# AppleHolic/pytorch_sound

Measured on AMD Instinct MI355X. Metric: audio-sec/s STFT+mel+fwd/bwd, higher is better.
Workload: dtype bf16; 1 GPU; configs[1]: Conv1d separator (4 x ResBlock1, C=256, on 513-bin magnitude), 22.05 kHz, STFT 1024/256, 80 mel, batch 32 x 2 s per GPU, Adam, bf16 autocast; global_batch=32, parallelism=dp1, model_params=5520386

## Files before the change

### include/psnd.h

```cpp
#ifndef PSND_H
#define PSND_H

#include <stdint.h>
#include <stddef.h>

#ifdef __cplusplus
extern "C" {
#endif

#define PSND_OK 0
#define PSND_E_ARG (-1)
#define PSND_E_SHAPE (-2)
#define PSND_E_HIP (-3)
#define PSND_E_UNSUPPORTED (-4)

#define PSND_FRAMING_CENTER 0
#define PSND_FRAMING_HIFIGAN 1
#define PSND_FRAMING_NONE 2

int psnd_version(void);
const char *psnd_last_error(void);
#ifdef PSND_LAB
void psnd_env_refresh(void);
#endif
// ... 65 lines not shown
typedef struct psnd_chain_pair {
    const void *W1;
    const float *bias1;
    float act1_slope;
    void *mid_out;
    const void *W2;
    const float *bias2;
    int off1, dstep1, off2, dstep2;
    float act2_slope;
    void *out_raw, *out_act;
    const void *M1, *M2;
    float m1_slope, m2_slope;
} psnd_chain_pair;
int psnd_conv1d_cl_chain_rows(int C, int k, int n_pairs, const int *taps);
int psnd_conv1d_cl_chain_plan(int C, int k, int n_pairs, const int *taps, int64_t R, int *mr_out);
int psnd_conv1d_cl_chain(const void *A, const void *res, const psnd_chain_pair *pairs, int n_pairs, int64_t N, int Lp, int L, int HP,
                         int C, int k, void *stream);
void psnd_conv_chain_stats(long long *out2);
int psnd_to_cl_nfk(const float *x_nfk, int64_t N, int K, int64_t F, int Lp, int HP, int Cp, int preop, void *out, void *stream);
int64_t psnd_mask_head_l1_blocks_nfk(int64_t N, int64_t F, int K);
int psnd_mask_head_l1_fwd_nfk(const void *y, const float *mag_nfk, const float *ref_nfk, int64_t N, int K, int64_t F, int Lp, int HP, int Cp,
                              float *est_nfk, double *part, void *stream);
int psnd_mask_head_l1_bwd_nfk(const float *gest_nfk, const float *mag_nfk, const void *y, const float *est_nfk, const float *ref_nfk,
                              const float *g, float coef, int64_t N, int K, int64_t F, int Lp, int HP, int Cp, void *gy, void *stream);
int psnd_mel_fwd_nfk(const float *mag_nfk, int64_t N, int64_t F, int M, int K, const void *mel_plan, int log_kind, float log_offset,
                     float pre_clamp_min, float clamp_lo, float clamp_hi, float *out, float *mel_lin, void *stream);
int psnd_mel_bwd_nfk(const float *gout, const float *mel_lin, int64_t N, int64_t F, int M, int K, const void *mel_plan, int log_kind,
                     float log_offset, float pre_clamp_min, float clamp_lo, float clamp_hi, float *gmag_nfk, void *stream);
int psnd_mel_l1_fwd_nfk(const float *mag_nfk, int64_t N, int64_t F, int M, int K, const void *mel_plan, int log_kind, float log_offset,
                        float pre_clamp_min, float clamp_lo, float clamp_hi, const float *ref, float *mel_lin, double *part, void *stream);
int psnd_mel_l1_bwd_nfk(const float *ref, const float *mel_lin, const float *g, float coef, int64_t N, int64_t F, int M, int K,
                        const void *mel_plan, int log_kind, float log_offset, float pre_clamp_min, float clamp_lo, float clamp_hi,
                        float *gmag_nfk, void *stream);
int64_t psnd_mask_head_l1_blocks(int64_t N, int64_t T, int Cp);
int psnd_mask_head_l1_fwd(const void *y, const float *mag, const float *ref, int64_t N, int C, int64_t T, int Lp, int HP, int Cp,
                          float *est, double *part, void *stream);
int psnd_mask_head_l1_bwd(const float *gest, const float *mag, const void *y, const float *est, const float *ref, const float *g,
                          float coef, int64_t N, int C, int64_t T, int Lp, int HP, int Cp, void *gy, void *stream);
int64_t psnd_mel_l1_blocks(int64_t N, int64_t F, int M);
int psnd_mel_l1_fwd(const float *mag, int64_t N, int64_t F, int M, int K, const void *mel_plan, int log_kind, float log_offset,
                    float pre_clamp_min, float clamp_lo, float clamp_hi, const float *ref, float *mel_lin, double *part, void *stream);
int psnd_mel_l1_bwd(const float *ref, const float *mel_lin, const float *g, float coef, int64_t N, int64_t F, int M, int K,
                    const void *mel_plan, int log_kind, float log_offset, float pre_clamp_min, float clamp_lo, float clamp_hi,
                    float *gmag, void *stream);
int psnd_nan_flag(const float *x, int64_t n, float *flag, void *stream);
int psnd_l1_loss_combine(const double *const *parts, const int64_t *nb, const double *scale, int terms, float *out, float *nan_flag, void *stream);
int psnd_conv_stats(int64_t *out4, int reset);
int psnd_conv_pair_stats(int64_t *out4, int reset);
int psnd_conv1d_cl_wgrad(const void *G1, const void *G2, const void *GM, float g2_slope, const void *xa, int64_t N,
                         int Lp, int Ca, int Cb, int k, int off0, int dstep, float *gw_part, float *gbias_part,
                         void *g_out, void *stream);
int psnd_conv1d_prep(const float *v, const float *g, const float *bias, int Cout, int Cin, int k, int Cb, int Ca,
                     void *wf, void *wb, float *bias_padded, void *stream);
int psnd_convtr1d_prep(const float *v, const float *g, const float *bias, int Cin, int Cout, int K, int stride, int Cr, int Cip,
                       void *wf, void *wb, float *bias_rep, void *stream);
int psnd_convtr1d_prep_multi(const void *descs_dev, int n, int total_blocks, void *stream);
int psnd_convtr1d_cl_fwd(const void *xa, const void *wf, const float *bias_rep, int64_t N, int Lp, int L, int HP, int Cip, int Cr,
                         int stride, int padding, int LpO, int HPO, float act_slope, void *out_raw, void *out_act, void *stream);
int psnd_convtr1d_cl_wgrad_splits(int64_t N, int Lp, int Cip, int Cr, int stride);
int psnd_convtr1d_cl_bwd(const void *g_raw, const void *g_act, const void *act, float act_slope, const void *wb, const void *xa,
                         int64_t N, int Lp, int L, int HP, int Cip, int Cr, int stride, int padding, int LpO, int HPO, void *gx,
                         void *g_eff, float *gw_part, void *stream);
int psnd_convtr1d_wnorm_bwd(const float *gw_part, int splits, const float *v, const float *g, int Cin, int Cout, int K, int stride,
                            int Cr, int Cip, float *gv, float *gg, void *stream);
int psnd_cl_mean_act_fwd(const void *a, const void *b, const void *c, const void *d, int count, float slope, void *out, int64_t n,
                         void *stream);
// ... 162 lines not shown
```

### pytorch_sound_amd/_lib.py

```python
import ctypes
import os
import numpy as np

_HERE = os.path.dirname(os.path.abspath(__file__))
LIB_PATH = os.environ.get('PSND_LIB', os.path.join(_HERE, 'libpsnd_hip.so'))

PSND_OK = 0
FRAMING_CENTER = 0
FRAMING_HIFIGAN = 1
FRAMING_NONE = 2
LOG_NONE, LOG_E, LOG_10 = 0, 1, 2

_c = ctypes
_P = _c.c_void_p
_I64 = _c.c_int64
_INT = _c.c_int
_F = _c.c_float
_D = _c.c_double
_U32 = _c.c_uint32
_U64 = _c.c_uint64

SIGNATURES = {
    'psnd_version': (_INT, []),
    'psnd_last_error': (_c.c_char_p, []),
# ... 18 lines not shown
    'psnd_conv1d_cl': (_INT, [_P, _P, _P, _F, _P, _P, _P, _P, _I64, _INT, _INT, _INT, _INT, _INT, _INT, _INT, _INT, _F, _F, _P, _P, _P, _P]),
    'psnd_conv1d_cl_pair_supported': (_INT, [_INT, _INT, _INT, _INT, _INT, _INT]),
    'psnd_conv1d_cl_pair': (_INT, [_P, _P, _P, _P, _F, _F, _P, _P, _P, _P, _F, _P, _I64, _INT, _INT, _INT, _INT, _INT, _INT, _INT, _INT, _INT, _F, _P, _P, _P]),
    'psnd_conv1d_cl_wgrad': (_INT, [_P, _P, _P, _F, _P, _I64, _INT, _INT, _INT, _INT, _INT, _INT, _P, _P, _P, _P]),
    'psnd_conv1d_prep': (_INT, [_P, _P, _P, _INT, _INT, _INT, _INT, _INT, _P, _P, _P, _P]),
    'psnd_conv1d_wnorm_bwd': (_INT, [_P, _P, _INT, _P, _P, _INT, _INT, _INT, _INT, _INT, _P, _P, _P, _P]),
    'psnd_conv1d_cl_bwd': (_INT, [_P, _P, _P, _F, _P, _P, _I64, _INT, _INT, _INT, _INT, _INT, _INT, _INT, _INT, _P, _P, _P, _F, _P, _P, _P, _P]),
    'psnd_conv1d_cl_wgrad_multi_splits': (_INT, [_I64, _INT, _INT, _INT, _INT, _INT]),
    'psnd_conv1d_cl_wgrad_multi': (_INT, [_P, _INT, _I64, _INT, _P]),
    'psnd_nan_flag': (_INT, [_P, _I64, _P, _P]),
    'psnd_conv1d_cl_chain_rows': (_INT, [_INT, _INT, _INT, _P]),
    'psnd_conv1d_cl_chain_plan': (_INT, [_INT, _INT, _INT, _P, _I64, _P]),
    'psnd_conv1d_cl_chain': (_INT, [_P, _P, _P, _INT, _I64, _INT, _INT, _INT, _INT, _INT, _P]),
    'psnd_conv_chain_stats': (None, [_P]),
    'psnd_conv1d_cl_pair_bwd_supported': (_INT, [_INT, _INT, _INT, _INT, _INT, _INT]),
    'psnd_conv1d_cl_pair_bwd_splits': (_INT, [_I64, _INT, _INT, _INT]),
    'psnd_conv1d_cl_pair_bwd': (_INT, [_P, _P, _P, _F, _P, _P, _P, _F, _P, _I64, _INT, _INT, _INT, _INT, _INT, _INT, _INT, _INT, _INT, _P, _P, _P, _P,
                                       _P, _P, _INT, _INT, _P, _P, _P]),
    'psnd_conv1d_wnorm_bwd_multi': (_INT, [_P, _INT, _P]),
    'psnd_conv1d_prep_multi': (_INT, [_P, _INT, _INT, _INT, _INT, _P]),
    'psnd_conv1d_cl_wgrad_splits': (_INT, [_I64, _INT, _INT, _INT, _INT]),
    'psnd_mask_head_l1_blocks': (_I64, [_I64, _I64, _INT]),
    'psnd_masked_l1_blocks': (_I64, [_I64]),
    'psnd_masked_l1_fwd': (_INT, [_P, _P, _P, _I64, _INT, _I64, _P, _P, _P, _P]),
    'psnd_masked_l1_bwd': (_INT, [_P, _P, _P, _I64, _INT, _I64, _P, _P, _P, _P, _P]),
    'psnd_to_cl_nfk': (_INT, [_P, _I64, _INT, _I64, _INT, _INT, _INT, _INT, _P, _P]),
    'psnd_mask_head_l1_blocks_nfk': (_I64, [_I64, _I64, _INT]),
    'psnd_mask_head_l1_fwd_nfk': (_INT, [_P, _P, _P, _I64, _INT, _I64, _INT, _INT, _INT, _P, _P, _P]),
    'psnd_mask_head_l1_bwd_nfk': (_INT, [_P, _P, _P, _P, _P, _P, _F, _I64, _INT, _I64, _INT, _INT, _INT, _P, _P]),
    'psnd_mel_fwd_nfk': (_INT, [_P, _I64, _I64, _INT, _INT, _P, _INT, _F, _F, _F, _F, _P, _P, _P]),
    'psnd_mel_bwd_nfk': (_INT, [_P, _P, _I64, _I64, _INT, _INT, _P, _INT, _F, _F, _F, _F, _P, _P]),
    'psnd_mel_l1_fwd_nfk': (_INT, [_P, _I64, _I64, _INT, _INT, _P, _INT, _F, _F, _F, _F, _P, _P, _P, _P]),
    'psnd_mel_l1_bwd_nfk': (_INT, [_P, _P, _P, _F, _I64, _I64, _INT, _INT, _P, _INT, _F, _F, _F, _F, _P, _P]),
    'psnd_mask_head_l1_fwd': (_INT, [_P, _P, _P, _I64, _INT, _I64, _INT, _INT, _INT, _P, _P, _P]),
    'psnd_mask_head_l1_bwd': (_INT, [_P, _P, _P, _P, _P, _P, _F, _I64, _INT, _I64, _INT, _INT, _INT, _P, _P]),
    'psnd_mel_l1_blocks': (_I64, [_I64, _I64, _INT]),
    'psnd_mel_l1_fwd': (_INT, [_P, _I64, _I64, _INT, _INT, _P, _INT, _F, _F, _F, _F, _P, _P, _P, _P]),
    'psnd_mel_l1_bwd': (_INT, [_P, _P, _P, _F, _I64, _I64, _INT, _INT, _P, _INT, _F, _F, _F, _F, _P, _P]),
    'psnd_l1_loss_combine': (_INT, [_P, _P, _P, _INT, _P, _P, _P]),
    'psnd_conv_stats': (_INT, [_P, _INT]),
    'psnd_conv_pair_stats': (_INT, [_P, _INT]),
    'psnd_convtr1d_prep_multi': (_INT, [_P, _INT, _INT, _P]),
    'psnd_convtr1d_prep': (_INT, [_P, _P, _P, _INT, _INT, _INT, _INT, _INT, _INT, _P, _P, _P, _P]),
    'psnd_convtr1d_cl_fwd': (_INT, [_P, _P, _P, _I64, _INT, _INT, _INT, _INT, _INT, _INT, _INT, _INT, _INT, _F, _P, _P, _P]),
    'psnd_convtr1d_cl_wgrad_splits': (_INT, [_I64, _INT, _INT, _INT, _INT]),
    'psnd_convtr1d_cl_bwd': (_INT, [_P, _P, _P, _F, _P, _P, _I64, _INT, _INT, _INT, _INT, _INT, _INT, _INT, _INT, _INT, _P, _P, _P, _P]),
    'psnd_convtr1d_wnorm_bwd': (_INT, [_P, _INT, _P, _P, _INT, _INT, _INT, _INT, _INT, _INT, _P, _P, _P]),
    'psnd_cl_mean_act_fwd': (_INT, [_P, _P, _P, _P, _INT, _F, _P, _I64, _P]),
    'psnd_cl_mean_act_bwd': (_INT, [_P, _P, _INT, _F, _P, _I64, _P]),
    'psnd_cl_sum2': (_INT, [_P, _INT, _P, _P, _INT, _P, _I64, _P]),
    'psnd_grad_pack_bf16': (_INT, [_P, _P, _I64, _F, _P]),
    'psnd_grad_unpack_bf16': (_INT, [_P, _P, _I64, _F, _P]),
    'psnd_cl_colsum_splits': (_INT, [_I64, _INT]),
    'psnd_cl_colsum': (_INT, [_P, _I64, _INT, _INT, _INT, _INT, _P, _P, _P]),
    'psnd_posenc': (_INT, [_P, _P, _F, _I64, _INT, _I64, _I64, _P, _P]),
    'psnd_groupnorm1_fwd': (_INT, [_P, _P, _P, _P, _I64, _INT, _I64, _F, _INT, _P, _P, _P, _P]),
    'psnd_groupnorm1_bwd': (_INT, [_P, _P, _P, _P, _P, _P, _I64, _INT, _I64, _INT, _P, _P, _P, _P, _P]),
    'psnd_groupnorm1_drop_fwd': (_INT, [_P, _P, _P, _P, _I64, _INT, _I64, _F, _INT, _P, _P, _P, _P, _U32, _F, _P]),
    'psnd_groupnorm1_drop_bwd': (_INT, [_P, _P, _P, _P, _P, _P, _I64, _INT, _I64, _INT, _P, _P, _P, _P, _P, _P, _U32, _F, _P]),
    'psnd_rng_seed': (_INT, [_P, _U64, _U64, _P]),
    'psnd_rng_next': (_INT, [_P, _P, _P]),
    'psnd_linear1x1_fwd': (_INT, [_P, _P, _P, _I64, _INT, _INT, _I64, _INT, _INT, _P, _P]),
    'psnd_linear1x1_wgrad_slabs': (_I64, [_I64, _INT, _INT, _I64]),
    'psnd_linear1x1_bwd': (_INT, [_P, _P, _P, _P, _I64, _INT, _INT, _I64, _INT, _P, _P, _P, _P, _P]),
    'psnd_linear1x1_bwd_acc': (_INT, [_P, _P, _P, _P, _I64, _INT, _INT, _I64, _INT, _P, _P, _P, _P, _P, _P]),
    'psnd_linear1x1_bwd_ex': (_INT, [_P, _P, _P, _P, _I64, _INT, _INT, _I64, _INT, _INT, _I64, _P, _P, _P, _P, _P, _P, _P]),
# ... 172 lines not shown
```

### pytorch_sound_amd/cl.py

```python
import ctypes
import os
from pytorch_sound_amd import _switches as _sw
import weakref

import torch

from . import _lib
from ._lib import lib, check, ptr, stream_ptr

ALIGN_C = 32


def round_up(x, m):
    return (x + m - 1) // m * m


class CLShape:

    def __init__(self, N, L, HP):
        self.N, self.L, self.HP = int(N), int(L), int(HP)
        self.Lp = round_up(self.L + 2 * self.HP, 8)

    @property
    def R(self):
# ... 168 lines not shown
    def backward(ctx, g, _gest):
        y, mag, mag_ref, mel_ref, mel_plan, est, lin = ctx.saved_tensors
        shape, M, log_kind, log_offset, pre, lo, hi, c1, c2 = ctx.cfg
        N, C, T = mag.shape
        if g is None:
            return (None,) * 14
        g = g.contiguous().float()
        gest = torch.empty_like(mag)
        gy = torch.empty_like(y)
        st = stream_ptr(y.device)
        with torch.cuda.device(y.device):
            check(lib().psnd_mel_l1_bwd(ptr(mel_ref), ptr(lin), ptr(g), c2, N, T, M, C, ptr(mel_plan), log_kind, log_offset, pre, lo, hi,
                                        ptr(gest), st), 'psnd_mel_l1_bwd')
            check(lib().psnd_mask_head_l1_bwd(ptr(gest), ptr(mag), ptr(y), ptr(est), ptr(mag_ref), ptr(g), c1, N, C, T, shape.Lp, shape.HP,
                                              y.shape[2], ptr(gy), st), 'psnd_mask_head_l1_bwd')
        return (gy,) + (None,) * 13


def to_cl_nfk(x_nfk, shape, preop=0):
    _need(x_nfk, torch.float32)
    if x_nfk.requires_grad and torch.is_grad_enabled():
        raise _lib.PsndError('to_cl_nfk carries no gradient (feature tensors are inputs); use ToCL on an (N, K, F) tensor')
    N, F, K = x_nfk.shape
    if F != shape.L or N != shape.N:
        raise _lib.PsndError('to_cl_nfk: tensor %s does not match the CL geometry (N=%d, L=%d)' % (tuple(x_nfk.shape), shape.N, shape.L))
    Cp = round_up(K, ALIGN_C)
    out = torch.empty((N, shape.Lp, Cp), dtype=torch.bfloat16, device=x_nfk.device)
    with torch.cuda.device(x_nfk.device):
        check(lib().psnd_to_cl_nfk(ptr(x_nfk), N, K, F, shape.Lp, shape.HP, Cp, int(preop), ptr(out), stream_ptr(x_nfk.device)),
              'psnd_to_cl_nfk')
    return out


class MaskHeadSpectralL1NFK(torch.autograd.Function):

    @staticmethod
    def forward(ctx, y, mag, mag_ref, mel_ref, mel_plan, shape, M, log_kind, log_offset, pre_clamp_min, clamp_lo, clamp_hi, w1, w2):
        from .kernels import _clamp_args
        ctx.set_materialize_grads(False)
        _need(y, torch.bfloat16)
        for t in (mag, mag_ref, mel_ref):
            _need(t, torch.float32)
        N, F, K = mag.shape
        if mag_ref.shape != mag.shape or tuple(mel_ref.shape) != (N, M, F):
            raise _lib.PsndError('mask_head_spectral_l1 (nfk): mag_ref %s / mel_ref %s do not match mag %s and %d mel bands'
                                 % (tuple(mag_ref.shape), tuple(mel_ref.shape), tuple(mag.shape), M))
        dev = y.device
        lo, hi, pre = _clamp_args(clamp_lo, clamp_hi, pre_clamp_min)
        est = torch.empty_like(mag)
        lin = torch.empty((N, M, F), dtype=torch.float32, device=dev)
        nb1 = int(lib().psnd_mask_head_l1_blocks_nfk(N, F, K))
        nb2 = int(lib().psnd_mel_l1_blocks(N, F, M))
        part = torch.empty(nb1 + nb2, dtype=torch.float64, device=dev)
        out = torch.empty((), dtype=torch.float32, device=dev)
        st = stream_ptr(dev)
        with torch.cuda.device(dev):
            check(lib().psnd_mask_head_l1_fwd_nfk(ptr(y), ptr(mag), ptr(mag_ref), N, K, F, shape.Lp, shape.HP, y.shape[2], ptr(est),
                                                  ptr(part), st), 'psnd_mask_head_l1_fwd_nfk')
            p2 = ctypes.c_void_p(part.data_ptr() + 8 * nb1)
            check(lib().psnd_mel_l1_fwd_nfk(ptr(est), N, F, M, K, ptr(mel_plan), log_kind, float(log_offset), pre, lo, hi, ptr(mel_ref),
                                            ptr(lin), p2, st), 'psnd_mel_l1_fwd_nfk')
            parts = (ctypes.c_void_p * 2)(part.data_ptr(), part.data_ptr() + 8 * nb1)
            nbs = (ctypes.c_int64 * 2)(nb1, nb2)
            sc = (ctypes.c_double * 2)(float(w1) / mag.numel(), float(w2) / mel_ref.numel())
            nan_flag = _nan_flag_tensor(dev)
            check(lib().psnd_l1_loss_combine(parts, nbs, sc, 2, ptr(out), ptr(nan_flag), st), 'psnd_l1_loss_combine')
        LAST_LOSS_NAN_FLAG[0] = nan_flag
        ctx.cfg = (shape, M, log_kind, float(log_offset), pre, lo, hi, float(w1) / mag.numel(), float(w2) / mel_ref.numel())
        ctx.save_for_backward(y, mag, mag_ref, mel_ref, mel_plan, est, lin)
        ctx.mark_non_differentiable(est)
        return out, est

    @staticmethod
    def backward(ctx, g, _gest):
        y, mag, mag_ref, mel_ref, mel_plan, est, lin = ctx.saved_tensors
        shape, M, log_kind, log_offset, pre, lo, hi, c1, c2 = ctx.cfg
        N, F, K = mag.shape
        if g is None:
            return (None,) * 14
        g = g.contiguous().float()
        gest = torch.empty_like(mag)
        gy = torch.empty_like(y)
        st = stream_ptr(y.device)
        with torch.cuda.device(y.device):
            check(lib().psnd_mel_l1_bwd_nfk(ptr(mel_ref), ptr(lin), ptr(g), c2, N, F, M, K, ptr(mel_plan), log_kind, log_offset, pre, lo, hi,
                                            ptr(gest), st), 'psnd_mel_l1_bwd_nfk')
            check(lib().psnd_mask_head_l1_bwd_nfk(ptr(gest), ptr(mag), ptr(y), ptr(est), ptr(mag_ref), ptr(g), c1, N, K, F, shape.Lp,
                                                  shape.HP, y.shape[2], ptr(gy), st), 'psnd_mask_head_l1_bwd_nfk')
        return (gy,) + (None,) * 13


def _launch_conv(A, A2, AM, a2_slope, W, bias, res, mask_src, shape, Ca, Cb, k, off0, dstep, act_slope, mask_slope,
                 want_raw, want_act, a_eff_out=None):
    dev = W.device
    raw = torch.empty((shape.N, shape.Lp, Cb), dtype=torch.bfloat16, device=dev) if want_raw else None
    act = torch.empty((shape.N, shape.Lp, Cb), dtype=torch.bfloat16, device=dev) if want_act else None
    with torch.cuda.device(dev):
        check(lib().psnd_conv1d_cl(ptr(A), ptr(A2), ptr(AM), float(a2_slope), ptr(W), ptr(bias), ptr(res), ptr(mask_src),
                                   shape.N, shape.Lp, shape.L, shape.HP, Ca, Cb, k, off0, dstep, float(act_slope),
                                   float(mask_slope), ptr(raw), ptr(act), ptr(a_eff_out), stream_ptr(dev)), 'psnd_conv1d_cl')
    return raw, act


_JOIN_PENDING = {}


def _join_side_at_end_of_backward(dev, side):
    target = torch.cuda.current_stream(dev)
    pending = _JOIN_PENDING.setdefault(dev.index, [])
    if not any(t == target and sd == side for t, sd in pending):
        pending.append((target, side))

    def join():
        for t, sd in _JOIN_PENDING.pop(dev.index, []):
            t.wait_stream(sd)

# ... 1019 lines not shown
```

### pytorch_sound_amd/csrc/psnd_core.hip

```cpp
#include "psnd_common.h"

static thread_local char g_err[512] = "";

void psnd_set_error(const char *fmt, ...) {
    va_list ap;
    va_start(ap, fmt);
    vsnprintf(g_err, sizeof(g_err), fmt, ap);
    va_end(ap);
}

extern "C" int psnd_version(void) { return 140; }

extern "C" const char *psnd_last_error(void) { return g_err; }

#ifdef PSND_LAB
std::atomic<int> g_psnd_env_gen{0};
extern "C" void psnd_env_refresh(void) { g_psnd_env_gen.fetch_add(1, std::memory_order_acq_rel); }
#endif

static inline int64_t pad_of(int n_fft, int hop, int framing) {
    if (framing == PSND_FRAMING_NONE) return 0;
    return framing == PSND_FRAMING_CENTER ? n_fft / 2 : (n_fft - hop) / 2;
}

extern "C" int64_t psnd_frame_count(int64_t T, int n_fft, int hop, int framing) {
    if (T <= 0 || n_fft <= 0 || hop <= 0) return 0;
    const int64_t L = T + 2 * pad_of(n_fft, hop, framing);
    if (L < n_fft) return 0;
    return (L - n_fft) / hop + 1;
}

extern "C" int64_t psnd_frame_sample_index(int64_t f, int m, int64_t T, int n_fft, int hop, int framing) {
    int64_t i = f * hop - pad_of(n_fft, hop, framing) + m;
    if (i < 0) i = -i;
    if (i >= T) i = 2 * (T - 1) - i;
    return i;
}

extern "C" void *psnd_event_create(void) {
    hipEvent_t ev = nullptr;
    if (hipEventCreateWithFlags(&ev, hipEventDisableTiming) != hipSuccess) {
        psnd_set_error("event_create: %s", hipGetErrorString(hipGetLastError()));
        return nullptr;
    }
// ... 96 lines not shown
```

### pytorch_sound_amd/csrc/psnd_mel.hip

```cpp
#include "psnd_common.h"
#include <math.h>
#include <string.h>
#include <vector>

namespace {

inline int hdr_ints(int MT, int KT) { return (8 + 2 * MT + 2 * KT + 63) & ~63; }

struct MelParams {
    const float *in0;
    const float *in1;
    const int *plan;
    float *out;
    float *lin;
    long long F;
    int N, R, Cc;
    int RT, CS;
    int band_off;
    int w_off;
    int nft;
    int log_kind;
    float log_offset, pre_clamp_min, clamp_lo, clamp_hi;
    const float *l1_ref;
    double *l1_part;
// ... 292 lines not shown
                        const f32x4 rf = *reinterpret_cast<const f32x4_u *>(p.l1_ref + o);
                        l1acc += fabsf(y.x - rf.x) + fabsf(y.y - rf.y) + fabsf(y.z - rf.z) + fabsf(y.w - rf.w);
                        *reinterpret_cast<f32x4_u *>(p.lin + o) = v;
                    } else {
                        for (int j = 0; j < 4; ++j)
                            if (f + j < F) {
                                l1acc += fabsf(y[j] - p.l1_ref[o + j]);
                                p.lin[o + j] = v[j];
                            }
                    }
                    continue;
                }
                if (f + 3 < F) {
                    *reinterpret_cast<f32x4_u *>(p.out + o) = y;
                    if (p.lin) *reinterpret_cast<f32x4_u *>(p.lin + o) = v;
                } else {
                    for (int j = 0; j < 4; ++j)
                        if (f + j < F) {
                            p.out[o + j] = y[j];
                            if (p.lin) p.lin[o + j] = v[j];
                        }
                }
            }
            if (p.l1_part) {
                double d = (double)l1acc;
#pragma unroll
                for (int m = 32; m >= 1; m >>= 1) d += __shfl_xor(d, m, 64);
                if (lane == 0) p.l1_part[wid * p.RT + T] = d;
            }
        }
    });
}

struct MelHostPlan {
    int M, K, MT, KS, KT, MS, hdr, fw_off, bw_off, wn_off, KS16, seg_off;
    size_t total_bytes;
};
MelHostPlan mel_layout(int M, int K) {
    MelHostPlan h;
    h.M = M, h.K = K;
    h.MT = (M + 15) / 16, h.KS = (K + 3) / 4;
    h.KT = (K + 15) / 16, h.MS = (M + 3) / 4;
    h.hdr = hdr_ints(h.MT, h.KT);
    h.fw_off = h.hdr;
    h.bw_off = h.fw_off + h.MT * h.KS * 64;
    h.KS16 = (K + 15) / 16;
    h.wn_off = h.bw_off + h.KT * h.MS * 64;
    h.seg_off = h.wn_off + h.MT * h.KS16 * 256;
    h.total_bytes = sizeof(float) * ((size_t)h.seg_off + 4 * h.MT + 4);
    return h;
}

}

extern "C" size_t psnd_mel_plan_bytes(int M, int K) {
    if (M <= 0 || K <= 0) return 0;
    return mel_layout(M, K).total_bytes;
}

extern "C" int psnd_mel_plan_build(int M, int K, const float *W, void *plan_host) {
    if (!W || !plan_host || M <= 0 || K <= 0) PSND_FAIL(PSND_E_ARG, "mel_plan_build: bad arguments");
    const MelHostPlan h = mel_layout(M, K);
    memset(plan_host, 0, h.total_bytes);
    int *hdr = static_cast<int *>(plan_host);
    float *fl = static_cast<float *>(plan_host);
    hdr[0] = M, hdr[1] = K, hdr[2] = h.MT, hdr[3] = h.KS, hdr[4] = h.KT, hdr[5] = h.MS;
// ... 126 lines not shown
}
extern "C" int psnd_mel_l1_bwd(const float *ref, const float *mel_lin, const float *g, float coef, int64_t N, int64_t F, int M, int K,
                               const void *mel_plan, int log_kind, float log_offset, float pre_clamp_min, float clamp_lo, float clamp_hi,
                               float *gmag, void *stream) {
    if (!g) PSND_FAIL(PSND_E_ARG, "mel_l1_bwd: null g");
    return mel_launch(true, ref, mel_lin, N, F, M, K, mel_plan, log_kind, log_offset, pre_clamp_min, clamp_lo, clamp_hi, gmag, nullptr,
                      stream, nullptr, nullptr, g, coef);
}

extern "C" int psnd_mel_fwd_nfk(const float *mag_nfk, int64_t N, int64_t F, int M, int K, const void *mel_plan, int log_kind, float log_offset,
                                float pre_clamp_min, float clamp_lo, float clamp_hi, float *out, float *mel_lin, void *stream) {
    return mel_launch(false, mag_nfk, nullptr, N, F, M, K, mel_plan, log_kind, log_offset, pre_clamp_min, clamp_lo, clamp_hi, out, mel_lin, stream,
                      nullptr, nullptr, nullptr, 0.f, true);
}
extern "C" int psnd_mel_bwd_nfk(const float *gout, const float *mel_lin, int64_t N, int64_t F, int M, int K, const void *mel_plan, int log_kind,
                                float log_offset, float pre_clamp_min, float clamp_lo, float clamp_hi, float *gmag_nfk, void *stream) {
    return mel_launch(true, gout, mel_lin, N, F, M, K, mel_plan, log_kind, log_offset, pre_clamp_min, clamp_lo, clamp_hi, gmag_nfk, nullptr, stream,
                      nullptr, nullptr, nullptr, 0.f, true);
}
extern "C" int psnd_mel_l1_fwd_nfk(const float *mag_nfk, int64_t N, int64_t F, int M, int K, const void *mel_plan, int log_kind, float log_offset,
                                   float pre_clamp_min, float clamp_lo, float clamp_hi, const float *ref, float *mel_lin, double *part,
                                   void *stream) {
    if (!ref || !mel_lin || !part) PSND_FAIL(PSND_E_ARG, "mel_l1_fwd_nfk: null ref / mel_lin / part");
    return mel_launch(false, mag_nfk, nullptr, N, F, M, K, mel_plan, log_kind, log_offset, pre_clamp_min, clamp_lo, clamp_hi, nullptr, mel_lin,
                      stream, ref, part, nullptr, 0.f, true);
}
extern "C" int psnd_mel_l1_bwd_nfk(const float *ref, const float *mel_lin, const float *g, float coef, int64_t N, int64_t F, int M, int K,
                                   const void *mel_plan, int log_kind, float log_offset, float pre_clamp_min, float clamp_lo, float clamp_hi,
                                   float *gmag_nfk, void *stream) {
    if (!g) PSND_FAIL(PSND_E_ARG, "mel_l1_bwd_nfk: null g");
    return mel_launch(true, ref, mel_lin, N, F, M, K, mel_plan, log_kind, log_offset, pre_clamp_min, clamp_lo, clamp_hi, gmag_nfk, nullptr,
                      stream, nullptr, nullptr, g, coef, true);
}
```

Before: 96750 audio-s/s.

## Fuse mask head, spectral L1, mel projection and mel L1 into single fwd/bwd kernels

Adds fused forward and backward kernels covering the mask-head sigmoid, the spectral L1 loss, the mel MFMA projection with log/clamp and the mel L1 loss. The forward kernel also does the final loss reduction and combine through a last-block ticket counter. This replaces several separate launches and the intermediate est/gest round-trips through memory with one launch per direction. The cost is more complex kernels with redundant overlapping loads, per-stream ticket state that must stay correct across calls, and a per-wave double reduction.

```diff
diff --git a/include/psnd.h b/include/psnd.h
--- a/include/psnd.h
+++ b/include/psnd.h
@@ -121,6 +121,15 @@
 int psnd_mel_l1_bwd_nfk(const float *ref, const float *mel_lin, const float *g, float coef, int64_t N, int64_t F, int M, int K,
                         const void *mel_plan, int log_kind, float log_offset, float pre_clamp_min, float clamp_lo, float clamp_hi,
                         float *gmag_nfk, void *stream);
+int64_t psnd_mask_mel_l1_parts(int64_t N, int64_t F, int M);
+int psnd_mask_mel_l1_fwd_nfk(const void *y, const float *mag_nfk, const float *ref_nfk, const float *mel_ref, int64_t N, int K, int64_t F, int M,
+                             int Lp, int HP, int Cp, const void *mel_plan, int log_kind, float log_offset, float pre_clamp_min, float clamp_lo,
+                             float clamp_hi, double scale1, double scale2, float *est_nfk, float *mel_lin, double *part, unsigned *ticket,
+                             float *out, float *nan_flag, void *stream);
+int psnd_mask_mel_l1_bwd_nfk(const float *mag_nfk, const void *y, const float *est_nfk, const float *ref_nfk, const float *mel_ref,
+                             const float *mel_lin, const float *g, float coef1, float coef2, int64_t N, int K, int64_t F, int M, int Lp, int HP,
+                             int Cp, const void *mel_plan, int log_kind, float log_offset, float pre_clamp_min, float clamp_lo, float clamp_hi,
+                             void *gy, void *stream);
 int64_t psnd_mask_head_l1_blocks(int64_t N, int64_t T, int Cp);
 int psnd_mask_head_l1_fwd(const void *y, const float *mag, const float *ref, int64_t N, int C, int64_t T, int Lp, int HP, int Cp,
                           float *est, double *part, void *stream);
diff --git a/pytorch_sound_amd/_lib.py b/pytorch_sound_amd/_lib.py
--- a/pytorch_sound_amd/_lib.py
+++ b/pytorch_sound_amd/_lib.py
@@ -74,6 +74,10 @@
     'psnd_mel_bwd_nfk': (_INT, [_P, _P, _I64, _I64, _INT, _INT, _P, _INT, _F, _F, _F, _F, _P, _P]),
     'psnd_mel_l1_fwd_nfk': (_INT, [_P, _I64, _I64, _INT, _INT, _P, _INT, _F, _F, _F, _F, _P, _P, _P, _P]),
     'psnd_mel_l1_bwd_nfk': (_INT, [_P, _P, _P, _F, _I64, _I64, _INT, _INT, _P, _INT, _F, _F, _F, _F, _P, _P]),
+    'psnd_mask_mel_l1_parts': (_I64, [_I64, _I64, _INT]),
+    'psnd_mask_mel_l1_fwd_nfk': (_INT, [_P, _P, _P, _P, _I64, _INT, _I64, _INT, _INT, _INT, _INT, _P, _INT, _F, _F, _F, _F, _D, _D, _P, _P, _P, _P, _P, _P,
+                                        _P]),
+    'psnd_mask_mel_l1_bwd_nfk': (_INT, [_P, _P, _P, _P, _P, _P, _P, _F, _F, _I64, _INT, _I64, _INT, _INT, _INT, _INT, _P, _INT, _F, _F, _F, _F, _P, _P]),
     'psnd_mask_head_l1_fwd': (_INT, [_P, _P, _P, _I64, _INT, _I64, _INT, _INT, _INT, _P, _P, _P]),
     'psnd_mask_head_l1_bwd': (_INT, [_P, _P, _P, _P, _P, _P, _F, _I64, _INT, _I64, _INT, _INT, _INT, _P, _P]),
     'psnd_mel_l1_blocks': (_I64, [_I64, _I64, _INT]),
diff --git a/pytorch_sound_amd/cl.py b/pytorch_sound_amd/cl.py
--- a/pytorch_sound_amd/cl.py
+++ b/pytorch_sound_amd/cl.py
@@ -224,6 +224,30 @@
     return out
 
 
+def loss_tail_fused() -> bool:
+    return os.environ.get('PSND_LOSS_TAIL') != 'unfused'
+
+
+_LOSS_TICKETS = {}
+_LOSS_TICKET_SLOTS = 64
+
+
+def _loss_ticket(dev):
+    stream = torch.cuda.current_stream(dev).cuda_stream
+    entry = _LOSS_TICKETS.get(dev.index)
+    if entry is None:
+        if torch.cuda.is_current_stream_capturing():
+            return torch.zeros(1, dtype=torch.int32, device=dev)
+        entry = _LOSS_TICKETS[dev.index] = (torch.zeros(_LOSS_TICKET_SLOTS, dtype=torch.int32, device=dev), {})
+    words, slots = entry
+    slot = slots.get(stream)
+    if slot is None:
+        if len(slots) == _LOSS_TICKET_SLOTS:
+            return torch.zeros(1, dtype=torch.int32, device=dev)
+        slot = slots[stream] = len(slots)
+    return words[slot:slot + 1]
+
+
 class MaskHeadSpectralL1NFK(torch.autograd.Function):
 
     @staticmethod
@@ -241,6 +265,22 @@
         lo, hi, pre = _clamp_args(clamp_lo, clamp_hi, pre_clamp_min)
         est = torch.empty_like(mag)
         lin = torch.empty((N, M, F), dtype=torch.float32, device=dev)
+        ctx.fused = loss_tail_fused()
+        if ctx.fused:
+            part = torch.empty(max(int(lib().psnd_mask_mel_l1_parts(N, F, M)), 1), dtype=torch.float64, device=dev)
+            out = torch.empty((), dtype=torch.float32, device=dev)
+            with torch.cuda.device(dev):
+                ticket = _loss_ticket(dev)
+                nan_flag = _nan_flag_tensor(dev)
+                check(lib().psnd_mask_mel_l1_fwd_nfk(ptr(y), ptr(mag), ptr(mag_ref), ptr(mel_ref), N, K, F, M, shape.Lp, shape.HP, y.shape[2],
+                                                     ptr(mel_plan), log_kind, float(log_offset), pre, lo, hi, float(w1) / mag.numel(),
+                                                     float(w2) / mel_ref.numel(), ptr(est), ptr(lin), ptr(part), ptr(ticket), ptr(out),
+                                                     ptr(nan_flag), stream_ptr(dev)), 'psnd_mask_mel_l1_fwd_nfk')
+            LAST_LOSS_NAN_FLAG[0] = nan_flag
+            ctx.cfg = (shape, M, log_kind, float(log_offset), pre, lo, hi, float(w1) / mag.numel(), float(w2) / mel_ref.numel())
+            ctx.save_for_backward(y, mag, mag_ref, mel_ref, mel_plan, est, lin)
+            ctx.mark_non_differentiable(est)
+            return out, est
         nb1 = int(lib().psnd_mask_head_l1_blocks_nfk(N, F, K))
         nb2 = int(lib().psnd_mel_l1_blocks(N, F, M))
         part = torch.empty(nb1 + nb2, dtype=torch.float64, device=dev)
@@ -271,9 +311,15 @@
         if g is None:
             return (None,) * 14
         g = g.contiguous().float()
-        gest = torch.empty_like(mag)
         gy = torch.empty_like(y)
         st = stream_ptr(y.device)
+        if ctx.fused:
+            with torch.cuda.device(y.device):
+                check(lib().psnd_mask_mel_l1_bwd_nfk(ptr(mag), ptr(y), ptr(est), ptr(mag_ref), ptr(mel_ref), ptr(lin), ptr(g), c1, c2, N, K, F, M,
+                                                     shape.Lp, shape.HP, y.shape[2], ptr(mel_plan), log_kind, log_offset, pre, lo, hi, ptr(gy),
+                                                     st), 'psnd_mask_mel_l1_bwd_nfk')
+            return (gy,) + (None,) * 13
+        gest = torch.empty_like(mag)
         with torch.cuda.device(y.device):
             check(lib().psnd_mel_l1_bwd_nfk(ptr(mel_ref), ptr(lin), ptr(g), c2, N, F, M, K, ptr(mel_plan), log_kind, log_offset, pre, lo, hi,
                                             ptr(gest), st), 'psnd_mel_l1_bwd_nfk')
diff --git a/pytorch_sound_amd/csrc/psnd_core.hip b/pytorch_sound_amd/csrc/psnd_core.hip
--- a/pytorch_sound_amd/csrc/psnd_core.hip
+++ b/pytorch_sound_amd/csrc/psnd_core.hip
@@ -9,7 +9,7 @@
     va_end(ap);
 }
 
-extern "C" int psnd_version(void) { return 140; }
+extern "C" int psnd_version(void) { return 141; }
 
 extern "C" const char *psnd_last_error(void) { return g_err; }
 
diff --git a/pytorch_sound_amd/csrc/psnd_mel.hip b/pytorch_sound_amd/csrc/psnd_mel.hip
--- a/pytorch_sound_amd/csrc/psnd_mel.hip
+++ b/pytorch_sound_amd/csrc/psnd_mel.hip
@@ -348,6 +348,335 @@
     });
 }
 
+typedef unsigned short bf16_t;
+typedef __bf16 hwbf16x2 __attribute__((ext_vector_type(2)));
+__device__ __forceinline__ float bf_lo(unsigned v) { return __builtin_bit_cast(float, v << 16); }
+__device__ __forceinline__ float bf_hi(unsigned v) { return __builtin_bit_cast(float, v & 0xffff0000u); }
+__device__ __forceinline__ unsigned pack_bf16(float lo, float hi) {
+    const f32x2 v = {lo, hi};
+    return __builtin_bit_cast(unsigned, __builtin_convertvector(v, hwbf16x2));
+}
+
+struct TailParams {
+    const bf16_t *y;
+    const float *mag, *ref;
+    float *est;
+    bf16_t *gy;
+    double *part;
+    unsigned *ticket;
+    float *loss, *nan_flag;
+    double scale1, scale2;
+    int Lp, HP, Cp;
+    float c1;
+};
+
+constexpr unsigned kOOB = 0xffffffffu;
+template <bool FULL>
+__device__ __forceinline__ f32x4 tail_load4(__amdgpu_buffer_rsrc_t r, unsigned off, int nv) {
+    if constexpr (FULL) {
+        return __builtin_bit_cast(f32x4, __builtin_amdgcn_raw_buffer_load_b128(r, (int)off, 0, 0));
+    } else {
+        f32x4 o;
+#pragma unroll
+        for (int j = 0; j < 4; ++j)
+            o[j] = __builtin_bit_cast(float, __builtin_amdgcn_raw_buffer_load_b32(r, (int)((off != kOOB && j < nv) ? off + 4u * j : kOOB), 0, 0));
+        return o;
+    }
+}
+__device__ __forceinline__ void tail_store4(__amdgpu_buffer_rsrc_t r, unsigned off, int nv, bool full, f32x4 v) {
+    if (full) {
+        __builtin_amdgcn_raw_buffer_store_b128(__builtin_bit_cast(u32x4, v), r, (int)off, 0, 0);
+    } else {
+#pragma unroll
+        for (int j = 0; j < 4; ++j)
+            __builtin_amdgcn_raw_buffer_store_b32(__builtin_bit_cast(unsigned, v[j]), r, (int)((off != kOOB && j < nv) ? off + 4u * j : kOOB), 0, 0);
+    }
+}
+__device__ __forceinline__ double wave_sum_d(double v) {
+#pragma unroll
+    for (int m = 32; m >= 1; m >>= 1) v += __shfl_xor(v, m, 64);
+    return v;
+}
+__device__ __forceinline__ double load_part(const double *p) {
+    return __builtin_bit_cast(double, __hip_atomic_load(reinterpret_cast<const unsigned long long *>(p), __ATOMIC_RELAXED, __HIP_MEMORY_SCOPE_AGENT));
+}
+
+__global__ __launch_bounds__(256) void mask_mel_fwd_kernel(MelParams p, TailParams q) {
+    const int lane = threadIdx.x & 63;
+    const long long wid = (long long)blockIdx.x * 4 + (threadIdx.x >> 6);
+    const long long per_clip = (long long)p.nft * p.RT;
+    const long long waves = per_clip * p.N;
+    if (wid < waves) {
+        const int clip = (int)(wid / per_clip);
+        const int rem = (int)(wid - (long long)clip * per_clip);
+        const int ft = rem / p.RT, rt = rem - ft * p.RT;
+        const long long F = p.F;
+        const long long f = (long long)ft * 64 + 4 * (lane & 15);
+        const int kk = lane >> 4;
+        const int K = p.Cc;
+        const int lo16 = p.plan[p.band_off + 2 * rt] >> 2, hi16 = (p.plan[p.band_off + 2 * rt + 1] + 3) >> 2;
+        int olo = 0, ohi = 0;
+        for (int t = 0; t <= rt; ++t) olo = ohi, ohi = max(ohi, (p.plan[p.band_off + 2 * t + 1] + 3) >> 2);
+        if (rt == p.RT - 1) ohi = p.CS16;
+        int wlo = lo16, whi = hi16;
+        if (ohi > olo) wlo = hi16 > lo16 ? min(lo16, olo) : olo, whi = hi16 > lo16 ? max(hi16, ohi) : ohi;
+        const f32x4 *Wn = reinterpret_cast<const f32x4 *>(reinterpret_cast<const float *>(p.plan) + p.wn_off) + (size_t)rt * p.CS16 * 64 + lane;
+        const int clip_bytes = (int)((size_t)K * F * sizeof(float));
+        const size_t clip_off = (size_t)clip * K * F;
+        const __amdgpu_buffer_rsrc_t rm = make_uniform_rsrc(q.mag + clip_off, clip_bytes), rr = make_uniform_rsrc(q.ref + clip_off, clip_bytes);
+        const __amdgpu_buffer_rsrc_t re = make_uniform_rsrc(q.est + clip_off, clip_bytes);
+        const __amdgpu_buffer_rsrc_t ry = make_uniform_rsrc(q.y + (size_t)clip * q.Lp * q.Cp, (int)((size_t)q.Lp * q.Cp * 2));
+        unsigned fb[4], yb[4];
+#pragma unroll
+        for (int g = 0; g < 4; ++g) {
+            fb[g] = (f + g < F) ? (unsigned)((((size_t)(f + g)) * K + 4 * kk) * sizeof(float)) : kOOB;
+            yb[g] = (f + g < F) ? (unsigned)((((size_t)(q.HP + f + g)) * q.Cp + 4 * kk) * 2) : kOOB;
+        }
+        f32x4 acc0 = {0.f, 0.f, 0.f, 0.f}, acc1 = acc0, acc2 = acc0, acc3 = acc0;
+        double sacc = 0.0;
+        for (int S0 = wlo; S0 < whi; S0 += 2) {
+            f32x4 a[2], mv[2][4], rv[2][4];
+            u32x2 yq[2][4];
+            bool bnd[2], own[2], full[2];
+#pragma unroll
+            for (int u = 0; u < 2; ++u) {
+                const int S = S0 + u;
+                bnd[u] = S >= lo16 && S < hi16, own[u] = S >= olo && S < ohi;
+                const bool in = bnd[u] || own[u];
+                full[u] = 16 * S + 16 <= K || !in;
+                a[u] = bnd[u] ? Wn[(size_t)S * 64] : f32x4{0.f, 0.f, 0.f, 0.f};
+                const int c = 16 * S + 4 * kk;
+                if (full[u]) {
+#pragma unroll
+                    for (int g = 0; g < 4; ++g) {
+                        const unsigned off = (in && fb[g] != kOOB) ? fb[g] + 64u * (unsigned)S : kOOB;
+                        mv[u][g] = tail_load4<true>(rm, off, 4);
+                        rv[u][g] = tail_load4<true>(rr, own[u] ? off : kOOB, 4);
+                    }
+                } else {
+#pragma unroll
+                    for (int g = 0; g < 4; ++g) {
+                        const unsigned off = fb[g] != kOOB ? fb[g] + 64u * (unsigned)S : kOOB;
+                        mv[u][g] = tail_load4<false>(rm, off, K - c);
+                        rv[u][g] = tail_load4<false>(rr, own[u] ? off : kOOB, K - c);
+                    }
+                }
+#pragma unroll
+                for (int g = 0; g < 4; ++g)
+                    yq[u][g] = __builtin_bit_cast(u32x2, __builtin_amdgcn_raw_buffer_load_b64(
+                        ry, (int)((in && yb[g] != kOOB && c < q.Cp) ? yb[g] + 32u * (unsigned)S : kOOB), 0, 0));
+            }
+#pragma unroll
+            for (int u = 0; u < 2; ++u) {
+                const int S = S0 + u;
+                const int c = 16 * S + 4 * kk;
+                f32x4 b[4];
+#pragma unroll
+                for (int g = 0; g < 4; ++g) {
+                    const bool cnt = own[u] && fb[g] != kOOB;
+                    float d[4];
+#pragma unroll
+                    for (int j = 0; j < 4; ++j) {
+                        const unsigned w = yq[u][g][j >> 1];
+                        const float yv = (j & 1) ? bf_hi(w) : bf_lo(w);
+                        float v = mv[u][g][j] / (1.f + __expf(-yv));
+                        if (c + j >= K) v = 0.f;
+                        b[g][j] = v;
+                        d[j] = __builtin_fabsf(v - rv[u][g][j]);
+                    }
+                    float h = 0.f;
+#pragma unroll
+                    for (int j = 0; j < 4; ++j)
+                        if (cnt && c + j < K) h += d[j];
+                    float t = __shfl_xor(h, 16, 64);
+#pragma unroll
+                    for (int j = 0; j < 4; ++j)
+                        if (cnt && c + j < K) t += d[j];
+                    sacc += (kk & 1) ? (double)t : 0.0;
+                    tail_store4(re, cnt ? fb[g] + 64u * (unsigned)S : kOOB, K - c, full[u], b[g]);
+                    if (!bnd[u]) b[g] = f32x4{0.f, 0.f, 0.f, 0.f};
+                }
+#pragma unroll
+                for (int j = 0; j < 4; ++j) {
+                    acc0 = __builtin_amdgcn_mfma_f32_16x16x4f32(a[u][j], b[0][j], acc0, 0, 0, 0);
+                    acc1 = __builtin_amdgcn_mfma_f32_16x16x4f32(a[u][j], b[1][j], acc1, 0, 0, 0);
+                    acc2 = __builtin_amdgcn_mfma_f32_16x16x4f32(a[u][j], b[2][j], acc2, 0, 0, 0);
+                    acc3 = __builtin_amdgcn_mfma_f32_16x16x4f32(a[u][j], b[3][j], acc3, 0, 0, 0);
+                }
+            }
+        }
+        const size_t obase = (size_t)clip * p.R * F;
+        float l1acc = 0.f;
+#pragma unroll
+        for (int r = 0; r < 4; ++r) {
+            const int row = 16 * rt + 4 * kk + r;
+            if (row >= p.R) continue;
+            const f32x4 v = {acc0[r], acc1[r], acc2[r], acc3[r]};
+            f32x4 yv;
+            yv.x = fminf(fmaxf(log_apply(v.x, p.log_kind, p.log_offset, p.pre_clamp_min), p.clamp_lo), p.clamp_hi);
+            yv.y = fminf(fmaxf(log_apply(v.y, p.log_kind, p.log_offset, p.pre_clamp_min), p.clamp_lo), p.clamp_hi);
+            yv.z = fminf(fmaxf(log_apply(v.z, p.log_kind, p.log_offset, p.pre_clamp_min), p.clamp_lo), p.clamp_hi);
+            yv.w = fminf(fmaxf(log_apply(v.w, p.log_kind, p.log_offset, p.pre_clamp_min), p.clamp_lo), p.clamp_hi);
+            const size_t o = obase + (size_t)row * F + f;
+            if (f + 3 < F) {
+                const f32x4 rf = *reinterpret_cast<const f32x4_u *>(p.l1_ref + o);
+                l1acc += fabsf(yv.x - rf.x) + fabsf(yv.y - rf.y) + fabsf(yv.z - rf.z) + fabsf(yv.w - rf.w);
+                *reinterpret_cast<f32x4_u *>(p.lin + o) = v;
+            } else {
+                for (int j = 0; j < 4; ++j)
+                    if (f + j < F) {
+                        l1acc += fabsf(yv[j] - p.l1_ref[o + j]);
+                        p.lin[o + j] = v[j];
+                    }
+            }
+        }
+        const double d1 = wave_sum_d(sacc), d2 = wave_sum_d((double)l1acc);
+        if (lane == 0) q.part[wid] = d1, q.part[waves + wid] = d2;
+    }
+    __threadfence();
+    __shared__ unsigned s_last;
+    __syncthreads();
+    if (threadIdx.x == 0) s_last = atomicAdd(q.ticket, 1u) == gridDim.x - 1 ? 1u : 0u;
+    __syncthreads();
+    if (!s_last) return;
+    __threadfence();
+    __shared__ double red[16];
+    const int nb = (int)waves;
+    for (int pass = 0; pass < 4; ++pass) {
+        const int vw = pass * 4 + (threadIdx.x >> 6), vt = vw * 64 + lane;
+        double s = 0;
+        for (int k = 0; k < 2; ++k) {
+            const double *part = q.part + (size_t)k * nb;
+            double sk = 0;
+            for (int i = vt; i < nb; i += 4096) {
+                double v[4];
+#pragma unroll
+                for (int u = 0; u < 4; ++u) v[u] = load_part(part + min(i + 1024 * u, nb - 1));
+#pragma unroll
+                for (int u = 0; u < 4; ++u) sk += i + 1024 * u < nb ? v[u] : 0.0;
+            }
+            s += sk * (k == 0 ? q.scale1 : q.scale2);
+        }
+        s = wave_sum_d(s);
+        if (lane == 0) red[vw] = s;
+    }
+    __syncthreads();
+    if (threadIdx.x == 0) {
+        double a = 0;
+        for (int w = 0; w < 16; ++w) a += red[w];
+        q.loss[0] = (float)a;
+        if (q.nan_flag) q.nan_flag[0] = a != a ? 1.f : 0.f;
+        __hip_atomic_store(q.ticket, 0u, __ATOMIC_RELAXED, __HIP_MEMORY_SCOPE_AGENT);
+    }
+}
+
+__global__ __launch_bounds__(256) void mask_mel_bwd_kernel(MelParams p, TailParams q) {
+    const int lane = threadIdx.x & 63;
+    const long long wid = (long long)blockIdx.x * 4 + (threadIdx.x >> 6);
+    const long long per_clip = (long long)p.nft * p.RT;
+    if (wid >= per_clip * p.N) return;
+    const int clip = (int)(wid / per_clip);
+    const int rem = (int)(wid - (long long)clip * per_clip);
+    const int ft = rem / p.RT, rt = rem - ft * p.RT;
+    const long long F = p.F;
+    const long long f = (long long)ft * 64 + 4 * (lane & 15);
+    const int kk = lane >> 4;
+    const int K = p.R;
+
+    const int lo = p.plan[p.band_off + 2 * rt], hi = p.plan[p.band_off + 2 * rt + 1];
+    const float *W = reinterpret_cast<const float *>(p.plan) + p.w_off + (size_t)rt * p.CS * 64 + lane;
+    const int in_bytes = (int)((size_t)p.Cc * F * sizeof(float));
+    const __amdgpu_buffer_rsrc_t r0 = make_uniform_rsrc(p.in0 + (size_t)clip * p.Cc * F, in_bytes);
+    const __amdgpu_buffer_rsrc_t r1 = make_uniform_rsrc(p.in1 + (size_t)clip * p.Cc * F, in_bytes);
+    const float g0 = p.l1_g[0];
+    const float l1c = p.l1_coef * g0;
+    f32x4 acc0 = {0.f, 0.f, 0.f, 0.f}, acc1 = acc0, acc2 = acc0, acc3 = acc0;
+    constexpr int MU = PSND_MEL_MU;
+    for (int s0 = lo; s0 < hi; s0 += MU) {
+        float a[MU];
+        f32x4 b[MU], m[MU];
+#pragma unroll
+        for (int u = 0; u < MU; ++u) {
+            const int c = s0 + u < hi ? 4 * (s0 + u) + kk : p.Cc;
+            a[u] = W[(size_t)min(s0 + u, hi - 1) * 64];
+            b[u] = load_b_raw(r0, c, p.Cc, f, F);
+            m[u] = load_b_raw(r1, c, p.Cc, f, F);
+        }
+#pragma unroll
+        for (int u = 0; u < MU; ++u) {
+            b[u].x = l1c * l1_log_grad(m[u].x, b[u].x, p.log_kind, p.log_offset, p.pre_clamp_min, p.clamp_lo, p.clamp_hi);
+            b[u].y = l1c * l1_log_grad(m[u].y, b[u].y, p.log_kind, p.log_offset, p.pre_clamp_min, p.clamp_lo, p.clamp_hi);
+            b[u].z = l1c * l1_log_grad(m[u].z, b[u].z, p.log_kind, p.log_offset, p.pre_clamp_min, p.clamp_lo, p.clamp_hi);
+            b[u].w = l1c * l1_log_grad(m[u].w, b[u].w, p.log_kind, p.log_offset, p.pre_clamp_min, p.clamp_lo, p.clamp_hi);
+            if (!(s0 + u < hi && 4 * (s0 + u) + kk < p.Cc)) b[u] = f32x4{0.f, 0.f, 0.f, 0.f};
+        }
+#pragma unroll
+        for (int u = 0; u < MU; ++u) {
+            acc0 = __builtin_amdgcn_mfma_f32_16x16x4f32(a[u], b[u].x, acc0, 0, 0, 0);
+            acc1 = __builtin_amdgcn_mfma_f32_16x16x4f32(a[u], b[u].y, acc1, 0, 0, 0);
+            acc2 = __builtin_amdgcn_mfma_f32_16x16x4f32(a[u], b[u].z, acc2, 0, 0, 0);
+            acc3 = __builtin_amdgcn_mfma_f32_16x16x4f32(a[u], b[u].w, acc3, 0, 0, 0);
+        }
+    }
+
+    const int bin0 = 16 * rt + 4 * kk;
+    const int clip_bytes = (int)((size_t)K * F * sizeof(float));
+    const size_t clip_off = (size_t)clip * K * F;
+    const __amdgpu_buffer_rsrc_t rm = make_uniform_rsrc(q.mag + clip_off, clip_bytes), rr = make_uniform_rsrc(q.ref + clip_off, clip_bytes);
+    const __amdgpu_buffer_rsrc_t re = make_uniform_rsrc(q.est + clip_off, clip_bytes);
+    const size_t cl0 = (size_t)clip * q.Lp * q.Cp;
+    const f32x4 accs[4] = {acc0, acc1, acc2, acc3};
+    const float sc = q.c1 * g0;
+    if (bin0 < q.Cp) {
+        const bool full = bin0 + 4 <= K;
+        f32x4 mv[4], ev[4], rv[4];
+        u32x2 yq[4];
+#pragma unroll
+        for (int j = 0; j < 4; ++j) {
+            const bool ok = f + j < F;
+            const unsigned off = ok && bin0 < K ? (unsigned)((((size_t)(f + j)) * K + bin0) * sizeof(float)) : kOOB;
+            if (full) mv[j] = tail_load4<true>(rm, off, 4), ev[j] = tail_load4<true>(re, off, 4), rv[j] = tail_load4<true>(rr, off, 4);
+            else mv[j] = tail_load4<false>(rm, off, K - bin0), ev[j] = tail_load4<false>(re, off, K - bin0), rv[j] = tail_load4<false>(rr, off, K - bin0);
+            yq[j] = ok ? *reinterpret_cast<const u32x2 *>(q.y + cl0 + (size_t)(q.HP + f + j) * q.Cp + bin0) : u32x2{0u, 0u};
+        }
+#pragma unroll
+        for (int j = 0; j < 4; ++j) {
+            if (f + j >= F) continue;
+            float w[4];
+#pragma unroll
+            for (int r = 0; r < 4; ++r) {
+                const unsigned yw = yq[j][r >> 1];
+                const float yv = (r & 1) ? bf_hi(yw) : bf_lo(yw);
+                const float sg = 1.f / (1.f + __expf(-yv));
+                const float d = ev[j][r] - rv[j][r];
+                const float gg = accs[j][r] + sc * (d > 0.f ? 1.f : (d < 0.f ? -1.f : 0.f));
+                w[r] = bin0 + r < K ? gg * mv[j][r] * sg * (1.f - sg) : 0.f;
+            }
+            *reinterpret_cast<u32x2 *>(q.gy + cl0 + (size_t)(q.HP + f + j) * q.Cp + bin0) = u32x2{pack_bf16(w[0], w[1]), pack_bf16(w[2], w[3])};
+        }
+    }
+    const u32x2 z2 = {0u, 0u};
+    const int ctop = 16 * p.RT;
+    if (rt == p.RT - 1 && ctop < q.Cp) {
+        const int quads = (q.Cp - ctop) >> 2;
+        for (int it = lane; it < 64 * quads; it += 64) {
+            const int fr = it / quads, qd = it - fr * quads;
+            const long long t = (long long)ft * 64 + fr;
+            if (t < F) *reinterpret_cast<u32x2 *>(q.gy + cl0 + (size_t)(q.HP + t) * q.Cp + ctop + 4 * qd) = z2;
+        }
+    }
+    if (ft == 0) {
+        const int c_lo = 16 * rt, c_hi = rt == p.RT - 1 ? q.Cp : min(16 * rt + 16, q.Cp);
+        const int quads = c_hi > c_lo ? (c_hi - c_lo) >> 2 : 0;
+        const int halo = q.Lp - (int)F;
+        for (int it = lane; it < halo * quads; it += 64) {
+            const int h = it / quads, qd = it - h * quads;
+            const int l = h < q.HP ? h : h + (int)F;
+            *reinterpret_cast<u32x2 *>(q.gy + cl0 + (size_t)l * q.Cp + c_lo + 4 * qd) = z2;
+        }
+    }
+}
+
 struct MelHostPlan {
     int M, K, MT, KS, KT, MS, hdr, fw_off, bw_off, wn_off, KS16, seg_off;
     size_t total_bytes;
@@ -540,3 +869,67 @@
     return mel_launch(true, ref, mel_lin, N, F, M, K, mel_plan, log_kind, log_offset, pre_clamp_min, clamp_lo, clamp_hi, gmag_nfk, nullptr,
                       stream, nullptr, nullptr, g, coef, true);
 }
+
+static int tail_setup(const char *what, int64_t N, int K, int64_t F, int M, int Lp, int HP, int Cp, const void *plan, int log_kind, float log_offset,
+                      float pre, float lo, float hi, bool bwd, MelParams &p) {
+    if (N < 0 || K <= 0 || F <= 0 || M <= 0 || HP < 0 || Lp < F + 2 * HP || Cp < ((K + 7) & ~7) || Cp % 8 != 0 ||
+        (size_t)N * (size_t)K * (size_t)F * 4 >= ((size_t)1 << 32) - 64 || (size_t)Lp * Cp * 2 >= ((size_t)1 << 31) ||
+        N * (int64_t)Lp * (Cp / 8) >= ((int64_t)1 << 39) || (size_t)(M > K ? M : K) * (size_t)F * sizeof(float) >= ((size_t)1 << 31))
+        PSND_FAIL(PSND_E_SHAPE, "%s: N=%lld K=%d F=%lld M=%d Lp=%d HP=%d Cp=%d", what, (long long)N, K, (long long)F, M, Lp, HP, Cp);
+    if (log_kind < PSND_LOG_NONE || log_kind > PSND_LOG_10) PSND_FAIL(PSND_E_ARG, "%s: log_kind=%d", what, log_kind);
+    const MelHostPlan h = mel_layout(M, K);
+    p = MelParams{};
+    p.plan = static_cast<const int *>(plan);
+    p.F = F, p.N = (int)N;
+    p.log_kind = log_kind, p.log_offset = log_offset, p.pre_clamp_min = pre, p.clamp_lo = lo, p.clamp_hi = hi;
+    p.nft = (int)((F + 63) / 64);
+    p.wn_off = h.wn_off, p.CS16 = h.KS16, p.seg_off = h.seg_off;
+    if (!bwd) p.R = M, p.Cc = K, p.RT = h.MT, p.CS = h.KS, p.band_off = 8, p.w_off = h.fw_off;
+    else p.R = K, p.Cc = M, p.RT = h.KT, p.CS = h.MS, p.band_off = 8 + 2 * h.MT, p.w_off = h.bw_off;
+    if (((long long)N * p.nft * p.RT + 3) / 4 >= (1ll << 31)) PSND_FAIL(PSND_E_SHAPE, "%s: grid too large", what);
+    return PSND_OK;
+}
+
+extern "C" int64_t psnd_mask_mel_l1_parts(int64_t N, int64_t F, int M) { return 2 * psnd_mel_l1_blocks(N, F, M); }
+
+extern "C" int psnd_mask_mel_l1_fwd_nfk(const void *y, const float *mag_nfk, const float *ref_nfk, const float *mel_ref, int64_t N, int K, int64_t F,
+                                        int M, int Lp, int HP, int Cp, const void *mel_plan, int log_kind, float log_offset, float pre_clamp_min,
+                                        float clamp_lo, float clamp_hi, double scale1, double scale2, float *est_nfk, float *mel_lin, double *part,
+                                        unsigned *ticket, float *out, float *nan_flag, void *stream) {
+    if (!y || !mag_nfk || !ref_nfk || !mel_ref || !mel_plan || !est_nfk || !mel_lin || !part || !ticket || !out)
+        PSND_FAIL(PSND_E_ARG, "mask_mel_l1_fwd_nfk: null pointer");
+    if ((reinterpret_cast<uintptr_t>(y) & 15) != 0) PSND_FAIL(PSND_E_ARG, "mask_mel_l1_fwd_nfk: y is not 16-byte aligned");
+    MelParams p;
+    if (int rc = tail_setup("mask_mel_l1_fwd_nfk", N, K, F, M, Lp, HP, Cp, mel_plan, log_kind, log_offset, pre_clamp_min, clamp_lo, clamp_hi, false, p))
+        return rc;
+    if (N == 0) return PSND_OK;
+    p.lin = mel_lin, p.l1_ref = mel_ref;
+    TailParams q = {};
+    q.y = static_cast<const bf16_t *>(y), q.mag = mag_nfk, q.ref = ref_nfk, q.est = est_nfk, q.part = part, q.ticket = ticket;
+    q.loss = out, q.nan_flag = nan_flag, q.scale1 = scale1, q.scale2 = scale2, q.Lp = Lp, q.HP = HP, q.Cp = Cp;
+    const long long blocks = ((long long)N * p.nft * p.RT + 3) / 4;
+    hipLaunchKernelGGL(mask_mel_fwd_kernel, dim3((unsigned)blocks), dim3(256), 0, static_cast<hipStream_t>(stream), p, q);
+    PSND_CHECK_LAUNCH("mask_mel_l1_fwd_nfk");
+    return PSND_OK;
+}
+
+extern "C" int psnd_mask_mel_l1_bwd_nfk(const float *mag_nfk, const void *y, const float *est_nfk, const float *ref_nfk, const float *mel_ref,
+                                        const float *mel_lin, const float *g, float coef1, float coef2, int64_t N, int K, int64_t F, int M, int Lp,
+                                        int HP, int Cp, const void *mel_plan, int log_kind, float log_offset, float pre_clamp_min, float clamp_lo,
+                                        float clamp_hi, void *gy, void *stream) {
+    if (!mag_nfk || !y || !est_nfk || !ref_nfk || !mel_ref || !mel_lin || !g || !mel_plan || !gy) PSND_FAIL(PSND_E_ARG, "mask_mel_l1_bwd_nfk: null pointer");
+    if (((reinterpret_cast<uintptr_t>(y) | reinterpret_cast<uintptr_t>(gy)) & 15) != 0)
+        PSND_FAIL(PSND_E_ARG, "mask_mel_l1_bwd_nfk: y / gy are not 16-byte aligned");
+    MelParams p;
+    if (int rc = tail_setup("mask_mel_l1_bwd_nfk", N, K, F, M, Lp, HP, Cp, mel_plan, log_kind, log_offset, pre_clamp_min, clamp_lo, clamp_hi, true, p))
+        return rc;
+    if (N == 0) return PSND_OK;
+    p.in0 = mel_ref, p.in1 = mel_lin, p.l1_g = g, p.l1_coef = coef2;
+    TailParams q = {};
+    q.y = static_cast<const bf16_t *>(y), q.mag = mag_nfk, q.ref = ref_nfk, q.est = const_cast<float *>(est_nfk), q.gy = static_cast<bf16_t *>(gy);
+    q.Lp = Lp, q.HP = HP, q.Cp = Cp, q.c1 = coef1;
+    const long long blocks = ((long long)N * p.nft * p.RT + 3) / 4;
+    hipLaunchKernelGGL(mask_mel_bwd_kernel, dim3((unsigned)blocks), dim3(256), 0, static_cast<hipStream_t>(stream), p, q);
+    PSND_CHECK_LAUNCH("mask_mel_l1_bwd_nfk");
+    return PSND_OK;
+}
```

After: 93250 audio-s/s. -3.6%, worse.
